# NVlabs/FoundationPose

Measured on AMD Instinct MI355X. Metric: pose-hypotheses/sec (raster+refine+score), 252 hyp x 160x160 @ 640x480 RGB-D, higher is better.
Workload: dtype f16

## Files before the change

### foundationpose_amd/_lib.py

```python
import ctypes as C
import os

import torch

_HERE = os.path.dirname(os.path.abspath(__file__))
LIB_PATH = os.environ.get("FP_AMD_LIB") or os.path.join(_HERE, "csrc", "libfp_amd.so")
ABI_VERSION = 234
_lib = None

vp, ci, cf, cd, sz = C.c_void_p, C.c_int, C.c_float, C.c_double, C.c_size_t

SIGNATURES = {
    "fp_last_error": (C.c_char_p, []),
    "fp_version": (ci, []),
    "fp_mesh_create": (ci, [vp, vp, vp, vp, vp, vp, vp, ci, ci, ci, ci, C.POINTER(vp)]),
    "fp_mesh_destroy": (None, [vp]),
    "fp_mesh_set_create": (ci, [vp, ci, C.POINTER(vp)]),
    "fp_mesh_set_destroy": (None, [vp]),
    "fp_mesh_set_workspace_bytes": (sz, [vp, ci, ci, ci]),
    "fp_depth_erode": (ci, [vp, vp, ci, ci, ci, cf, cf, cf, vp]),
    "fp_depth_bilateral": (ci, [vp, vp, ci, ci, ci, cf, cf, cf, vp]),
    "fp_depth_to_xyz": (ci, [vp, vp, cf, ci, vp, ci, ci, vp]),
    "fp_crop_windows": (ci, [vp, vp, vp, vp, ci, cd, vp, vp, ci, cd, ci, ci, ci, vp, vp, vp]),
    "fp_depth_erode_frames": (ci, [vp, vp, ci, ci, ci, ci, cf, cf, cf, vp]),
# ... 22 lines not shown
    "fp_tsdf_count_triangles": (ci, [vp, vp, ci, ci, ci, cf, vp, vp]),
    "fp_tsdf_emit_triangles": (ci, [vp, vp, vp, vp, ci, ci, ci, vp, cf, cf, vp, C.c_longlong, vp, vp, vp, vp, vp]),
    "fp_tsdf_label_components": (ci, [vp, ci, ci, ci, vp, vp, vp]),
    "fp_tsdf_raycast": (ci, [vp, vp, vp, vp, ci, ci, ci, vp, cf, cf, vp, vp, vp, vp, ci, vp, ci, ci, ci, ci, ci, cf, cf, cf, vp, vp, vp, vp, vp]),
    "fp_texture_bake": (ci, [vp, ci, vp, ci, vp, vp, vp, vp, vp, vp, ci, ci, ci, ci, ci, cf, cf, cf, vp, vp, vp]),
    "fp_workspace_bytes": (sz, [ci, ci, ci, ci, ci]),
    "fp_raster_lds_bytes": (sz, [ci]),
    "fp_render_crops": (ci, [vp, vp, vp, vp, cf, vp, vp, vp, vp, vp, ci, ci, ci, ci, ci, ci, cf, cf, cf, ci, vp, vp, vp, vp, vp, vp, vp, vp, sz, vp]),
    "fp_warp_crops": (ci, [vp, vp, vp, vp, vp, vp, vp, ci, vp, cf, vp, vp, ci, ci, ci, ci, ci, ci, ci, ci, vp, vp]),
    "fp_pose_update": (ci, [vp, vp, vp, ci, ci, vp, cf, cf, vp, vp, ci, ci, vp, vp, vp, ci, vp, vp, vp, ci, vp, cf, vp]),
    "fp_conv7x7s2_bn_relu_fwd": (ci, [vp, vp, vp, vp, vp, vp, ci, ci, ci, ci, vp]),
    "fp_igemm_f16_fwd": (ci, [vp, vp, vp, vp, vp, ci, ci, ci, ci, vp, vp]),
    "fp_pack_conv3x3_tiles_f16": (ci, [vp, vp, ci, ci, vp]),
    "fp_pack_conv3x3_tiles_direct_f16": (ci, [vp, vp, ci, ci, vp]),
    "fp_conv3x3_sw_lds_bytes": (ci, []),
    "fp_igemm_splitk_workspace_bytes": (sz, [ci, ci, ci]),
    "fp_igemm_f16_splitk_fwd": (ci, [vp, vp, vp, vp, vp, ci, ci, ci, ci, vp, ci, vp, sz, vp]),
    "fp_add_pe_f16_fwd": (ci, [vp, vp, vp, ci, ci, ci, vp]),
    "fp_replicate_rows_f16": (ci, [vp, vp, ci, ci, ci, ci, ci, C.c_longlong, vp]),
    "fp_replicate_segments_f16": (ci, [vp, vp, ci, ci, ci, ci, ci, C.c_longlong, vp]),
    "fp_layernorm_res_fwd": (ci, [vp, vp, vp, ci, vp, vp, vp, cf, vp, vp, ci, ci, vp]),
    "fp_pack_linear512_f16": (ci, [vp, vp, vp]),
    "fp_linear512_f16_fwd": (ci, [vp, vp, vp, vp, ci, ci, ci, vp]),
    "fp_linear_layernorm_fwd": (ci, [vp, vp, vp, vp, vp, vp, ci, vp, vp, cf, vp, vp, ci, ci, ci, ci, vp]),
    "fp_ffn_layernorm_mean_fwd": (ci, [vp, vp, vp, vp, vp, vp, vp, vp, cf, vp, vp, C.c_size_t, ci, ci, vp]),
    "fp_encoder_tail_workspace_bytes": (sz, [ci, ci]),
    "fp_encoder_tail_mean_fwd": (ci, [vp, ci, vp, vp, vp, vp, vp, vp, vp, vp, vp, vp, vp, vp, cf, vp, vp, sz, ci, ci, vp]),
    "fp_colmean_f16_fwd": (ci, [vp, vp, vp, vp, cf, vp, ci, ci, ci, vp]),
    "fp_rows_linear_fwd": (ci, [vp, vp, vp, vp, ci, ci, ci, ci, vp]),
    "fp_attention_f16_fwd": (ci, [vp, vp, ci, ci, ci, ci, ci, vp]),
    "fp_attention_segments_f16_fwd": (ci, [vp, vp, vp, ci, ci, ci, ci, ci, vp]),
    "fp_cluster_poses": (ci, [cf, cf, vp, ci, vp, ci, vp]),
}


class FpAmdError(RuntimeError):
    pass


def lib():
    global _lib
    if _lib is None:
        if not os.path.exists(LIB_PATH):
            raise FpAmdError(
                f"{LIB_PATH} is missing: the HIP extension is not built (run __graft_entry__.build() or "
                f"`make -C foundationpose_amd/csrc`). There is no CPU fallback.")
# ... 18 lines not shown
```

### foundationpose_amd/csrc/linear_ln.hip

```cpp
#include <hip/hip_fp16.h>
#include <stdlib.h>
#include <string.h>
#include <type_traits>
#include "igemm_common.h"
#include "rowops_ln.h"

#ifdef FP_PROFILE_BUILD
__device__ unsigned long long ll_dbg[8];
extern "C" int fp_dbg_linear_ln(unsigned long long* out, int reset) {
  if (reset) { unsigned long long z[8] = {0, 0, 0, 0, 0, 0, ~0ull, 0}; return (int)hipMemcpyToSymbol(HIP_SYMBOL(ll_dbg), z, sizeof(z)); }
  return (int)hipMemcpyFromSymbol(out, HIP_SYMBOL(ll_dbg), 8 * sizeof(unsigned long long));
}
#define LL_CLK(t) const unsigned long long t = wall_clock64()
#else
#define LL_CLK(t)
#endif

namespace {

constexpr int LL_BM = 128, LL_BN = 512, LL_K = 512, LL_NW = 8, LL_THREADS = LL_NW * 64, LL_BK = 32;
constexpr int LL_NK = LL_K / LL_BK;
constexpr int LL_KK = LL_BK / 16;
constexpr int LL_TM = LL_BM / 32;
constexpr int LL_ROWB = LL_BK * 2;
// ... 7 lines not shown

struct LinearLnParams {
  const _Float16* X;
  const _Float16* Wp;
  const float* bias;
  const float* x32;
  const _Float16* tok16;
  const float* pe;
  int S;
  const float* gamma;
  const float* beta;
  float eps;
  float* y32;
  _Float16* y16;
  int M;
  int ldx;
  float* part;
  const _Float16* W2p;
  const float* bias2;
  const _Float16* W1p;
  const float* bias1;
};

__global__ __launch_bounds__(256) void k_pack_w512(const _Float16* __restrict__ W, _Float16* __restrict__ out, int K) {
  const int o = blockIdx.x * 256 + threadIdx.x;
  const int lane = o & 63, i = (o >> 6) & 1, rest = o >> 7, nq = K / 16;
  const int q = rest % nq, w = rest / nq;
  if (w >= LL_BN / 64) return;
  const half8 v = *reinterpret_cast<const half8*>(W + (size_t)(64 * w + 32 * i + (lane & 31)) * K + 16 * q + 8 * (lane >> 5));
  *reinterpret_cast<half8*>(out + (size_t)o * 8) = v;
}

__device__ __forceinline__ int ll_swz(int row) { return (row >> 2) & 3; }

__device__ __forceinline__ void ll_dma16(const __amdgpu_buffer_rsrc_t& rs, void* lds, int voff, int soff) {
  __builtin_amdgcn_raw_ptr_buffer_load_lds(rs, (__attribute__((address_space(3))) void*)lds, 16, voff, soff, 0, 0);
}

__device__ __forceinline__ void ll_wait_vm(int n) {
  switch (n) {
    case 0: asm volatile("s_waitcnt vmcnt(0)" ::: "memory"); break;
    case 1: asm volatile("s_waitcnt vmcnt(1)" ::: "memory"); break;
    case 2: asm volatile("s_waitcnt vmcnt(2)" ::: "memory"); break;
    case 4: asm volatile("s_waitcnt vmcnt(4)" ::: "memory"); break;
    case 5: asm volatile("s_waitcnt vmcnt(5)" ::: "memory"); break;
    case 6: asm volatile("s_waitcnt vmcnt(6)" ::: "memory"); break;
    case 8: asm volatile("s_waitcnt vmcnt(8)" ::: "memory"); break;
    case 9: asm volatile("s_waitcnt vmcnt(9)" ::: "memory"); break;
    case 10: asm volatile("s_waitcnt vmcnt(10)" ::: "memory"); break;
    default: asm volatile("s_waitcnt vmcnt(0)" ::: "memory"); break;
  }
}
// ... 295 lines not shown
    const int mrow = m0 + wid * LL_ROWS_PER_WAVE;
    if (mrow < p.M) store8f(p.part + (size_t)(mrow / LL_ROWS_PER_WAVE) * 512 + lane * 8, csum);
  }
#ifdef FP_PROFILE_BUILD
  asm volatile("s_waitcnt vmcnt(0)" ::: "memory");
  LL_CLK(t_end);
  if (tid == 0) {
    atomicAdd(&ll_dbg[0], t_loop1 - t_start); atomicAdd(&ll_dbg[1], t_loop2 - t_pre); atomicAdd(&ll_dbg[2], t_park - t_loop2);
    atomicAdd(&ll_dbg[3], t_end - t_park); atomicAdd(&ll_dbg[4], 1ull); atomicMin(&ll_dbg[6], t_start); atomicMax(&ll_dbg[7], t_end);
  }
#endif
}

struct Linear512Params {
  const _Float16* X;
  const _Float16* Wp;
  const float* bias;
  _Float16* Y;
  int M, N, relu;
};
constexpr int L5_XBUF = 32 * 64;
constexpr int L5_BIAS_OFF = LL_E_BYTES + LL_NW * L5_XBUF;
constexpr int L5_MAX_N = 3072;
constexpr int l5_lds(int N) { return L5_BIAS_OFF + N * 4; }
static_assert(l5_lds(L5_MAX_N) <= 160 * 1024, "tile does not fit the 160 KiB LDS");

__global__ __launch_bounds__(LL_THREADS, 1) void k_linear512(Linear512Params p) {
  extern __shared__ __attribute__((aligned(16))) unsigned char smem[];
  const int tid = threadIdx.x, lane = tid & 63;
  const int wid = __builtin_amdgcn_readfirstlane(tid >> 6);
  float* bias_lds = reinterpret_cast<float*>(smem + L5_BIAS_OFF);
  unsigned char* xbuf = smem + LL_E_BYTES + wid * L5_XBUF;
  const int m0 = blockIdx.x * LL_BM;
  const int nblk = p.N / LL_BN;

  for (int q = wid; q < p.N / 256; q += LL_NW) {
    float* dst = bias_lds + q * 256;
    if (p.bias) {
      const __amdgpu_buffer_rsrc_t rs = __builtin_amdgcn_make_buffer_rsrc(const_cast<float*>(p.bias), 0, p.N * 4, 0x00020000);
      ll_dma16(rs, dst, lane * 16, q * 1024);
    } else {
      *reinterpret_cast<float4_*>(dst + lane * 4) = float4_{0.f, 0.f, 0.f, 0.f};
    }
  }
  unsigned aoff32;
  {
    const int row = wid * 16 + lane / 4;
    const int c = (lane % 4) ^ ll_swz(row);
    int m = m0 + row;
    m = m < p.M ? m : p.M - 1;
    aoff32 = (unsigned)(((size_t)m * LL_K + c * 8) * 2);
  }
  const __amdgpu_buffer_rsrc_t rsA = __builtin_amdgcn_make_buffer_rsrc(const_cast<_Float16*>(p.X), 0, 0x7FFFFFFF, 0x00020000);
  auto request_a = [&](int ks) { ll_dma16(rsA, smem + ks * LL_A_BLOCK + wid * 1024, (int)aoff32, ks * (LL_BK * 2)); };
  half8 wr[LL_LW + 1][LL_KK][2];
  auto request_w = [&](const _Float16* wp, int ks, int slot) {
    const _Float16* src = wp + ((size_t)wid * (LL_K / 16) + ks * LL_KK) * 1024 + lane * 8;
#pragma unroll
    for (int kk = 0; kk < LL_KK; ++kk)
#pragma unroll
      for (int i = 0; i < 2; ++i) wr[slot][kk][i] = *reinterpret_cast<const half8*>(src + (kk * 2 + i) * 512);
  };
  float16_ acc[2][LL_TM];
  const int frow = lane & 31, fhalf = lane >> 5;
  const unsigned char* a_ptr[2][LL_KK];
#pragma unroll
  for (int kk = 0; kk < LL_KK; ++kk) {
    a_ptr[0][kk] = smem + frow * LL_ROWB + (((2 * kk + fhalf) ^ ll_swz(frow)) << 4);
    a_ptr[1][kk] = a_ptr[0][kk] + 8 * LL_A_BLOCK;
  }
  half8 fa[2][LL_TM];
  auto read_a = [&](int ks, int kk, int slot) {
#pragma unroll
    for (int t = 0; t < LL_TM; ++t)
      fa[slot][t] = *reinterpret_cast<const half8*>(a_ptr[ks >> 3][kk] + (ks & 7) * LL_A_BLOCK + t * 32 * LL_ROWB);
  };
  auto mfma_group = [&](int wslot, int kk, int aslot) {
#pragma unroll
    for (int i = 0; i < 2; ++i)
#pragma unroll
      for (int j = 0; j < LL_TM; ++j)
        acc[i][j] = __builtin_amdgcn_mfma_f32_32x32x16_f16(wr[wslot][kk][i], fa[aslot][j], acc[i][j], 0, 0, 0);
  };
  auto zero_acc = [&]() {
#pragma unroll
    for (int i = 0; i < 2; ++i)
#pragma unroll
      for (int j = 0; j < LL_TM; ++j)
#pragma unroll
        for (int e = 0; e < 16; ++e) acc[i][j][e] = 0.f;
  };
  auto store_block = [&](int nb) {
    const half4 zero4 = {0, 0, 0, 0};
#pragma unroll
    for (int i = 0; i < 2; ++i) {
      const int nl = nb * LL_BN + wid * 64 + i * 32;
#pragma unroll
      for (int j = 0; j < LL_TM; ++j) {
#pragma unroll
        for (int g = 0; g < 4; ++g) {
          const float4_ bv = *reinterpret_cast<const float4_*>(bias_lds + nl + 8 * g + 4 * fhalf);
          half4 v;
#pragma unroll
          for (int e = 0; e < 4; ++e) v[e] = (_Float16)(acc[i][j][g * 4 + e] + bv[e]);
          if (p.relu) v = __builtin_elementwise_max(v, zero4);
          *reinterpret_cast<half4*>(xbuf + frow * 64 + ((g ^ ll_swz(frow)) << 4) + 8 * fhalf) = v;
        }
        __builtin_amdgcn_s_waitcnt(0xc07f);
        __builtin_amdgcn_wave_barrier();
#pragma unroll
        for (int h = 0; h < 2; ++h) {
          const int r = h * 16 + (lane >> 2), c = lane & 3;
          const half8 o = *reinterpret_cast<const half8*>(xbuf + r * 64 + ((c ^ ll_swz(r)) << 4));
          const int m = m0 + j * 32 + r;
          if (m < p.M) *reinterpret_cast<half8*>(p.Y + (size_t)m * p.N + nl + c * 8) = o;
        }
        __builtin_amdgcn_s_waitcnt(0xc07f);
        __builtin_amdgcn_wave_barrier();
      }
    }
  };

  zero_acc();
#pragma unroll
  for (int j = 0; j < LL_LA - LL_LW; ++j) request_a(j);
#pragma unroll
  for (int j = 0; j < LL_LW; ++j) { request_a(j + LL_LA - LL_LW); request_w(p.Wp, j, j); }
  ll_wait_vm(ll_after_w(0));
  __builtin_amdgcn_s_barrier();
  read_a(0, 0, 0);
#pragma unroll
  for (int ks = 0; ks < LL_NK; ++ks) {
    if (ks + LL_LA < LL_NK) request_a(ks + LL_LA);
    if (ks + LL_LW < LL_NK) request_w(p.Wp, ks + LL_LW, (ks + LL_LW) % (LL_LW + 1));
    read_a(ks, 1, 1);
    __builtin_amdgcn_sched_barrier(0);
    mfma_group(ks % (LL_LW + 1), 0, 0);
    __builtin_amdgcn_sched_barrier(0);
    if (ks + 1 < LL_NK) {
      ll_wait_vm(ll_after_w(ks + 1));
      __builtin_amdgcn_s_barrier();
      read_a(ks + 1, 0, 0);
    }
// ... 9 lines not shown
#pragma unroll 1
  for (int nb = 1; nb < nblk; ++nb) {
    const _Float16* wp = p.Wp + (size_t)nb * LL_BN * LL_K;
    zero_acc();
    read_a(0, 0, 0);
#pragma unroll
    for (int ks = 0; ks < LL_NK; ++ks) {
      if (ks + LL_LW < LL_NK) request_w(wp, ks + LL_LW, (ks + LL_LW) % (LL_LW + 1));
      read_a(ks, 1, 1);
      __builtin_amdgcn_sched_barrier(0);
      mfma_group(ks % (LL_LW + 1), 0, 0);
      __builtin_amdgcn_sched_barrier(0);
      if (ks + 1 < LL_NK) read_a(ks + 1, 0, 0);
      __builtin_amdgcn_sched_barrier(0);
      mfma_group(ks % (LL_LW + 1), 1, 1);
      __builtin_amdgcn_sched_barrier(0);
    }
    if (nb + 1 < nblk) {
#pragma unroll
      for (int j = 0; j < LL_LW; ++j) request_w(wp + (size_t)LL_BN * LL_K, j, j);
    }
    store_block(nb);
  }
}

__global__ __launch_bounds__(512) void k_ln_mean_finish(const float* __restrict__ part, const float* __restrict__ gamma,
                                                       const float* __restrict__ beta, float* __restrict__ out, int S) {
  const int g = blockIdx.x, c = threadIdx.x;
  const int nch = S / 16;
  const float* src = part + (size_t)g * nch * 512 + c;
  float a = 0.f;
  for (int k = 0; k < nch; ++k) a += src[(size_t)k * 512];
  a *= 1.0f / (float)S;
  out[(size_t)g * 512 + c] = fmaf(a, gamma[c], beta[c]);
}

}

extern "C" int fp_pack_linear512_f16(const void* w16, void* packed, void* stream) {
  FP_REQUIRE(w16 && packed, "fp_pack_linear512_f16: NULL tensor");
  FP_REQUIRE(w16 != packed, "fp_pack_linear512_f16: cannot pack in place");
  FP_REQUIRE((((size_t)w16 | (size_t)packed) & 15) == 0, "fp_pack_linear512_f16: tensors must be 16-byte aligned");
  hipLaunchKernelGGL(k_pack_w512, dim3(LL_BN * LL_K / 8 / 256), dim3(256), 0, (hipStream_t)stream, (const _Float16*)w16, (_Float16*)packed,
                     LL_K);
  FP_CHECK_LAUNCH("fp_pack_linear512_f16");
  return FP_OK;
}

extern "C" int fp_linear512_f16_fwd(const void* x16, const void* w_packed, const float* bias, void* y16, int M, int N, int relu,
                                    void* stream) {
  FP_REQUIRE(M >= 0, "fp_linear512_f16_fwd: M < 0");
  if (M == 0) return FP_OK;
  FP_REQUIRE(x16 && w_packed && y16, "fp_linear512_f16_fwd: NULL tensor");
  FP_REQUIRE(N >= LL_BN && N % LL_BN == 0 && N <= L5_MAX_N, "fp_linear512_f16_fwd: N=%d must be a multiple of 512, at most %d", N, L5_MAX_N);
  FP_REQUIRE((long long)M * N < (1ll << 31), "fp_linear512_f16_fwd: output exceeds 2^31 elements");
  FP_REQUIRE((((size_t)x16 | (size_t)w_packed | (size_t)bias | (size_t)y16) & 15) == 0, "fp_linear512_f16_fwd: tensors must be 16-byte aligned");
  Linear512Params p;
  p.X = (const _Float16*)x16; p.Wp = (const _Float16*)w_packed; p.bias = bias; p.Y = (_Float16*)y16; p.M = M; p.N = N; p.relu = relu ? 1 : 0;
  const int lds = l5_lds(N);
  FP_SET_MAX_LDS(k_linear512, l5_lds(L5_MAX_N));
  hipLaunchKernelGGL(k_linear512, dim3(fp_cdiv(M, LL_BM)), dim3(LL_THREADS), lds, (hipStream_t)stream, p);
  FP_CHECK_LAUNCH("fp_linear512_f16_fwd");
  return FP_OK;
}

extern "C" int fp_ffn_layernorm_mean_fwd(const void* y16, const void* w1_packed, const float* b1, const void* w2_packed, const float* b2,
                                         const float* x32, const float* gamma, const float* beta, float eps, float* out,
                                         float* workspace, size_t workspace_bytes, int groups, int rows_per_group, void* stream) {
  FP_REQUIRE(groups >= 0, "fp_ffn_layernorm_mean_fwd: groups < 0");
  if (groups == 0) return FP_OK;
  FP_REQUIRE(y16 && w1_packed && w2_packed && x32 && gamma && beta && out && workspace, "fp_ffn_layernorm_mean_fwd: NULL tensor");
  FP_REQUIRE(rows_per_group >= 16 && rows_per_group % 16 == 0,
             "fp_ffn_layernorm_mean_fwd: rows_per_group=%d must be a multiple of 16 (a wave sums 16 consecutive rows, which have to belong to one group)", rows_per_group);
  const long long M = (long long)groups * rows_per_group;
  FP_REQUIRE(M * 512 < (1ll << 30), "fp_ffn_layernorm_mean_fwd: operands exceed 2 GiB");
  FP_REQUIRE((((size_t)y16 | (size_t)w1_packed | (size_t)w2_packed | (size_t)b1 | (size_t)b2 | (size_t)x32 | (size_t)gamma | (size_t)beta) & 15) == 0,
             "fp_ffn_layernorm_mean_fwd: tensors must be 16-byte aligned");
  const int tiles = fp_cdiv((int)M, LL_BM);
  FP_REQUIRE(workspace_bytes >= (size_t)(M / 16) * 512 * sizeof(float), "fp_ffn_layernorm_mean_fwd: workspace too small");
  LinearLnParams p;
  p.X = (const _Float16*)y16; p.Wp = (const _Float16*)w1_packed; p.bias = b1; p.x32 = x32; p.tok16 = nullptr; p.pe = nullptr;
  p.S = rows_per_group; p.gamma = gamma; p.beta = beta; p.eps = eps; p.y32 = nullptr; p.y16 = nullptr; p.M = (int)M; p.ldx = LL_K;
  p.part = workspace; p.W2p = (const _Float16*)w2_packed; p.bias2 = b2; p.W1p = nullptr; p.bias1 = nullptr;
  FP_SET_MAX_LDS((k_rows512<true, true>), LL_LDS);
  hipLaunchKernelGGL((k_rows512<true, true>), dim3(tiles), dim3(LL_THREADS), LL_LDS, (hipStream_t)stream, p);
  hipLaunchKernelGGL(k_ln_mean_finish, dim3(groups), dim3(512), 0, (hipStream_t)stream, (const float*)workspace, gamma, beta, out,
// ... 69 lines not shown
```

### foundationpose_amd/engine.py

```python
import contextlib

import torch
import torch.nn.functional as F

from . import ops

USE_MIOPEN = False


FUSED_OUT_PROJ_LN = True


FUSED_FFN = True


ROWS_QKV = True
ROWS_QKV_MIN_ROWS = 4096
PACKED_CONV_TILES = True
MERGED_HEAD_QKV = True
FUSED_TAIL = True
CONV_MFMA_16X16X32 = True
SPECIALIZED_EPILOGUE = True
CONV_DIRECT_STORE = True


def _conv_backend():
    if USE_MIOPEN or not torch.backends.cudnn.is_available():
        return contextlib.nullcontext()
    return torch.backends.cudnn.flags(enabled=False)


def _bn_affine(sd, bn_p):
    if bn_p is None or (bn_p + ".weight") not in sd:
        return None, None
    scale = sd[bn_p + ".weight"].float() / torch.sqrt(sd[bn_p + ".running_var"].float() + 1e-5)
    shift = sd[bn_p + ".bias"].float() - sd[bn_p + ".running_mean"].float() * scale
    return scale.contiguous(), shift.contiguous()


def _r16(t):
    return t.to(torch.float16).to(torch.float32).contiguous()


class _Conv:

    def __init__(self, sd, conv_p, bn_p, stride, dtype, channels_last):
# ... 76 lines not shown

    def __call__(self, x):
        x = F.layer_norm(x + self.att(x), (x.shape[-1],), self.n1[0], self.n1[1], 1e-5)
        ff = F.linear(F.relu(F.linear(x, *self.l1)), *self.l2)
        return F.layer_norm(x + ff, (x.shape[-1],), self.n2[0], self.n2[1], 1e-5)


def _conv_params(sd, conv_p, bn_p, second_output=False):
    w = sd[conv_p + ".weight"].float()
    b = sd.get(conv_p + ".bias")
    scale, shift = _bn_affine(sd, bn_p)
    wk = w.permute(0, 2, 3, 1).reshape(w.shape[0], -1).to(torch.float16).contiguous()
    tiles, direct = None, bool(CONV_DIRECT_STORE and CONV_MFMA_16X16X32 and SPECIALIZED_EPILOGUE and b is not None and not second_output)
    if wk.is_cuda and w.shape[2] == 3 and w.shape[3] == 3 and w.shape[0] % 128 == 0 and w.shape[1] % 32 == 0 and PACKED_CONV_TILES:
        tiles = (ops.pack_conv3x3_tiles_direct if direct else ops.pack_conv3x3_tiles)(wk, w.shape[0], w.shape[1])
    return dict(w=wk, w_tiles=tiles, tiles_direct=direct and tiles is not None, bias=None if b is None else _r16(b.float()), scale=scale, shift=shift)


SPLITK_MAX_HYPS = 12
HEADS_TWO_STREAMS_MAX_HYPS = 12
SPLITK_TARGET_WGS = 384
SMALL_CALL_CEILING = 31

_SWITCHES = ("FUSED_OUT_PROJ_LN", "FUSED_FFN", "ROWS_QKV", "PACKED_CONV_TILES", "MERGED_HEAD_QKV", "FUSED_TAIL", "CONV_MFMA_16X16X32", "SPECIALIZED_EPILOGUE", "CONV_DIRECT_STORE", "SPLITK_MAX_HYPS", "HEADS_TWO_STREAMS_MAX_HYPS")


@contextlib.contextmanager
def overrides(**kw):
    g = globals()
    for k, v in kw.items():
        if k not in _SWITCHES:
            raise KeyError(f"engine.overrides: unknown switch {k!r} (known: {', '.join(_SWITCHES)})")
        if k.endswith("_MAX_HYPS") and not (0 <= int(v) <= SMALL_CALL_CEILING):
            raise ValueError(f"engine.overrides: {k} = {v} is outside 0..{SMALL_CALL_CEILING}")
    saved = {k: g[k] for k in kw}
    g.update(kw)
    try:
        yield
    finally:
        g.update(saved)


def small_call(n, limit):
    return n <= min(int(limit), SMALL_CALL_CEILING)


def splitk_pieces(rows, cout, cin):
# ... 108 lines not shown
        No = self.w.shape[0]
        y = torch.empty((M, No), dtype=torch.float16, device=x.device)
        Gm = ops.IgemmGeom.matrix
        ops.igemm_f16(x2, Gm(K), self.w, self.b, y, Gm(No), M, No, K, 1, relu=relu)
        return y.reshape(*x.shape[:-1], No)


class _HipRowsLinear:

    def __init__(self, w, b):
        self.w = w.to(torch.float16).contiguous()
        self.b = _r16(b.float())

    def __call__(self, x, round_f16=True, out_f16=False, out=None):
        return ops.rows_linear(x, self.w, self.b, round_f16=round_f16, out_f16=out_f16, out=out)


class _HipMHA:
    def __init__(self, sd, p, fp16_scores, nhead=4, small_calls=True):
        self.qkv = _HipLinear(sd[p + ".in_proj_weight"], sd[p + ".in_proj_bias"])
        self.out = _HipLinear(sd[p + ".out_proj.weight"], sd[p + ".out_proj.bias"])
        self.out_rows = _HipRowsLinear(sd[p + ".out_proj.weight"], sd[p + ".out_proj.bias"])
        self.nhead, self.fp16_scores = nhead, fp16_scores
        self.qkv_p = ops.PackedLinear512(self.qkv.w) if tuple(self.qkv.w.shape) == (1536, 512) else None
        self.small_calls = small_calls
        self._sk = {}

    def context(self, x16, slot=0, small_calls=True):
        Bn, L, D = x16.shape
        qkv = self.in_proj(x16, slot, small_calls)
        return ops.attention_f16(qkv.reshape(Bn, L, 3 * D), self.nhead, fp16_scores=self.fp16_scores)

    def in_proj(self, x16, slot=0, small_calls=True):
        Bn, L, D = x16.shape
        if ROWS_QKV and self.qkv_p is not None and Bn * L >= ROWS_QKV_MIN_ROWS:
            qkv = ops.linear512(x16, self.qkv_p, self.qkv.b)
        elif self.small_calls and small_calls and small_call(Bn, SPLITK_MAX_HYPS) and D % 64 == 0 and D // 64 >= 4:
            M, No = Bn * L, self.qkv.w.shape[0]
            pieces = max(1, min(D // 64 // 2, round(SPLITK_TARGET_WGS / (-(-M // 128) * (No // 128)))))
            key = (M, No, pieces, x16.device, slot)
            ws = self._sk.get(key)
            if ws is None:
                ws = self._sk[key] = torch.empty(ops.igemm_splitk_workspace_bytes(M, No, pieces), dtype=torch.uint8, device=x16.device)
            qkv = torch.empty((M, No), dtype=torch.float16, device=x16.device)
            Gm = ops.IgemmGeom.matrix
            ops.igemm_f16_splitk(x16.reshape(M, D), Gm(D), self.qkv.w, self.qkv.b, qkv, Gm(No), M, No, D, 1, pieces, ws)
        else:
# ... 42 lines not shown
    return {k: v.detach().to(device) for k, v in sd.items()}


class RefinePlan:
    small_calls = True

    def __init__(self, model, device, precision="fp16", channels_last=True):
        _check_precision(precision)
        self.dtype = torch.float16 if precision == "fp16" else torch.float32
        self.hip = self.dtype == torch.float16
        self.module = model if precision == "torch_amp" else None
        if self.module is not None:
            return
        sd = _dev_sd(model, device)
        self.heads = {}
        if self.hip:
            self.enc = _HipEncoder(sd, "encodeA", "encodeAB", device)
            for name in ("trans", "rot"):
                self.heads[name] = (_HipEncoderLayer(sd, f"{name}_head.0"),
                                    _HipRowsLinear(sd[f"{name}_head.1.weight"], sd[f"{name}_head.1.bias"]))
            wt, wr = (self.heads[n][0].att.qkv for n in ("trans", "rot"))
            if tuple(wt.w.shape) == (1536, 512) and tuple(wr.w.shape) == (1536, 512):
                cut = lambda t: (t[0:512], t[512:1024], t[1024:1536])
                self.qkv2_p = ops.PackedLinear512(torch.cat([p for pair in zip(cut(wt.w), cut(wr.w)) for p in pair], 0).contiguous())
                self.qkv2_b = torch.cat([p for pair in zip(cut(wt.b), cut(wr.b)) for p in pair], 0).contiguous()
            else:
                self.qkv2_p = None
        else:
            self.enc = _Encoder(sd, "encodeA", "encodeAB", self.dtype, channels_last)
            for name in ("trans", "rot"):
                self.heads[name] = (_TorchEncoderLayer(sd, f"{name}_head.0", self.dtype),
                                    sd[f"{name}_head.1.weight"].to(self.dtype), sd[f"{name}_head.1.bias"].to(self.dtype))

    def _head_side_stream(self, tok16):
        if not getattr(self, "two_stream_heads", True) or not self.small_calls or not small_call(tok16.shape[0], HEADS_TWO_STREAMS_MAX_HYPS) \
                or tok16.device.type != "cuda" or ops.KernelTimers.active is not None:
            return None
        from . import overlap
        if torch.cuda.is_current_stream_capturing() and not overlap.reserved(tok16.device, 1):
            return None
        if not overlap.side_streams_overlap(tok16.device, 1):
            return None
        return overlap.reserve_streams(tok16.device, 1)[0]

    @torch.inference_mode()
    def __call__(self, AB, slot=0, shared_b=False):
        out = {}
# ... 123 lines not shown
```

### foundationpose_amd/ops.py

```python
import ctypes as C
from typing import NamedTuple, Optional

import numpy as np
import torch

from . import _lib

FLAG_NORMALIZE_XYZ = 1
FLAG_OUT_F16 = 2
MODE_REFINE = 0
MODE_SCORE = 1
ROT_AXIS_ANGLE = 0
ROT_6D = 1
TRANS_TRACKNET, TRANS_DEEPIM, TRANS_RAW = 0, 1, 2


def _stream(t=None):
    if t is None:
        return C.c_void_p(torch.cuda.current_stream().cuda_stream)
    dev = t.device
    if dev.index is not None and dev.index != torch.cuda.current_device():
        raise _lib.FpAmdError(f"tensor on {dev} but the current device is cuda:{torch.cuda.current_device()}: wrap the call in "
                              f"`with torch.cuda.device({dev.index}):` (kernels launch on the current device)")
    return C.c_void_p(torch.cuda.current_stream(dev).cuda_stream)
# ... 1778 lines not shown
    _, Hp, Wp, Ct = (int(v) for v in buf.shape)
    st = _lib.lib().fp_replicate_segments_f16(C.c_void_p(buf.data_ptr() + 2 * int(c0)), _ptr(segments.dev), len(segments), n, Hp * Wp,
                                              int(c1) - int(c0), Ct, Hp * Wp * Ct, _stream(buf))
    _lib.check(st, "fp_replicate_segments_f16")
    return buf


def layernorm_res(branch16, gamma, beta, eps=1e-5, x32=None, tok16=None, pe=None, want32=True, want16=True):
    br = _dev(branch16, torch.float16, "branch16")
    D = int(br.shape[-1])
    M = br.numel() // D
    x32 = _dev(x32, torch.float32, "x32"); tok16 = _dev(tok16, torch.float16, "tok16"); pe = _dev(pe, torch.float32, "pe")
    S = int(pe.shape[-2]) if pe is not None else 0
    y32 = torch.empty(br.shape, dtype=torch.float32, device=br.device) if want32 else None
    y16 = torch.empty_like(br) if want16 else None
    st = _lib.lib().fp_layernorm_res_fwd(_ptr(x32), _ptr(tok16), _ptr(pe), S, _ptr(br), _ptr(_dev(gamma, torch.float32, "gamma")),
                                         _ptr(_dev(beta, torch.float32, "beta")), float(eps), _ptr(y32), _ptr(y16), M, D, _stream(br))
    _lib.check(st, "fp_layernorm_res_fwd")
    return y32, y16


class PackedLinear512:

    def __init__(self, w16):
        w = _dev(w16, torch.float16, "w16")
        if w.dim() != 2 or int(w.shape[1]) != 512 or int(w.shape[0]) % 512 or int(w.shape[0]) == 0:
            raise _lib.FpAmdError(f"PackedLinear512: weight {tuple(w.shape)}, must be (512 n, 512)")
        self.out_features = int(w.shape[0])
        self.data = torch.empty_like(w)
        for blk in range(self.out_features // 512):
            _lib.check(_lib.lib().fp_pack_linear512_f16(_ptr(w[blk * 512:]), _ptr(self.data[blk * 512:]), _stream(w)), "fp_pack_linear512_f16")


def _packed(w, name, out_features=512):
    if not isinstance(w, PackedLinear512):
        raise _lib.FpAmdError(f"{name}: the weight must be a PackedLinear512 (ops.PackedLinear512(w16))")
    if out_features is not None and w.out_features != out_features:
        raise _lib.FpAmdError(f"{name}: packed weight has {w.out_features} output features, expected {out_features}")
    return w.data


def linear512(x16, w_packed, bias, relu=False, out=None):
    x = _dev(x16, torch.float16, "x16")
    w = _packed(w_packed, "linear512", None)
    if int(x.shape[-1]) != 512:
        raise _lib.FpAmdError(f"linear512: x16 (..., {int(x.shape[-1])}), must be (..., 512)")
    N = w_packed.out_features
    M = x.numel() // 512
    y = out if out is not None else torch.empty(tuple(x.shape[:-1]) + (N,), dtype=torch.float16, device=x.device)
    if y.dtype != torch.float16 or y.numel() != M * N or not y.is_contiguous():
        raise _lib.FpAmdError("linear512: out must be a contiguous fp16 tensor of M x N elements")
    _lib.check(_lib.lib().fp_linear512_f16_fwd(_ptr(x), _ptr(w), _ptr(_dev(bias, torch.float32, "bias")), _ptr(y), M, N, 1 if relu else 0,
                                               _stream(x)), "fp_linear512_f16_fwd")
    return y


def linear_layernorm_res(x16, w_packed, bias, gamma, beta, eps=1e-5, x32=None, tok16=None, pe=None, want32=True, want16=True):
    w = _packed(w_packed, "linear_layernorm_res")
    if not (torch.is_tensor(x16) and x16.is_cuda and x16.dtype == torch.float16):
        raise _lib.FpAmdError("linear_layernorm_res: x16 must be a CUDA float16 tensor")
    K = int(x16.shape[-1])
    D = 512
    if K != 512:
        raise _lib.FpAmdError(f"linear_layernorm_res: x16 (..., {K}), must be (..., 512)")
    M = x16.numel() // K
    x, ldx = x16, _column_block(x16, "linear_layernorm_res: x16", sep="")
    x32 = _dev(x32, torch.float32, "x32"); tok16 = _dev(tok16, torch.float16, "tok16"); pe = _dev(pe, torch.float32, "pe")
    S = int(pe.shape[-2]) if pe is not None else 0
    shape = tuple(x.shape[:-1]) + (D,)
    y32 = torch.empty(shape, dtype=torch.float32, device=x.device) if want32 else None
    y16 = torch.empty(shape, dtype=torch.float16, device=x.device) if want16 else None
    st = _lib.lib().fp_linear_layernorm_fwd(_ptr(x), _ptr(w), _ptr(_dev(bias, torch.float32, "bias")), _ptr(x32), _ptr(tok16), _ptr(pe), S,
                                            _ptr(_dev(gamma, torch.float32, "gamma")), _ptr(_dev(beta, torch.float32, "beta")), float(eps),
                                            _ptr(y32), _ptr(y16), M, K, D, ldx, _stream(x))
    _lib.check(st, "fp_linear_layernorm_fwd")
    return y32, y16
# ... 301 lines not shown
```

### include/fp_amd.h

```cpp
#ifndef FP_AMD_H
#define FP_AMD_H

#include <stddef.h>
#include <stdint.h>

#ifdef __cplusplus
extern "C" {
#endif

typedef enum {
  FP_OK = 0,
  FP_ERR_INVALID_ARG = -1,
  FP_ERR_WORKSPACE = -2,
  FP_ERR_LAUNCH = -3,
  FP_ERR_UNSUPPORTED = -4
} fp_status;

#define FP_FLAG_NORMALIZE_XYZ 1
#define FP_FLAG_OUT_F16 2

#define FP_MODE_REFINE 0
#define FP_MODE_SCORE 1

#define FP_ROT_AXIS_ANGLE 0
// ... 209 lines not shown
size_t fp_igemm_splitk_workspace_bytes(int M, int N, int splits);
int fp_igemm_f16_splitk_fwd(const void* x , const fp_igemm_geom* x_geom , const void* w , void* y ,
                            const fp_igemm_geom* y_geom , int M, int N, int Cin, int taps,
                            const fp_igemm_epilogue* epilogue , int splits, void* workspace ,
                            size_t workspace_bytes, void* stream);

int fp_add_pe_f16_fwd(const void* tok , const float* pe , void* out , int M, int S, int D, void* stream);

int fp_replicate_rows_f16(const void* src , void* dst , int copies, int rows, int channels, int src_row_stride,
                          int dst_row_stride, long long dst_copy_stride, void* stream);

int fp_replicate_segments_f16(void* buf , const int32_t* seg_offsets , int segments, int images, int pixels,
                              int channels, int pixel_stride, long long image_stride, void* stream);

int fp_layernorm_res_fwd(const float* x32 , const void* tok16 , const float* pe , int S,
                         const void* branch16 , const float* gamma , const float* beta , float eps,
                         float* y32 , void* y16 , int M, int D, void* stream);

int fp_pack_linear512_f16(const void* w16 , void* packed , void* stream);

int fp_linear512_f16_fwd(const void* x16 , const void* w_packed , const float* bias , void* y16 ,
                         int M, int N, int relu, void* stream);

int fp_linear_layernorm_fwd(const void* x16 , const void* w16_packed , const float* bias ,
                            const float* x32 , const void* tok16 , const float* pe , int S,
                            const float* gamma , const float* beta , float eps, float* y32 ,
                            void* y16 , int M, int K, int D, int ldx ,
                            void* stream);

size_t fp_encoder_tail_workspace_bytes(int groups, int rows_per_group);
int fp_encoder_tail_mean_fwd(const void* ctx16 , int ldx, const void* wo_packed , const float* bo ,
                             const void* tok16 , const float* pe , const float* gamma1 , const float* beta1 ,
                             const void* w1_packed , const float* b1 , const void* w2_packed ,
                             const float* b2 , const float* gamma2 , const float* beta2 , float eps,
                             float* out , void* workspace , size_t workspace_bytes, int groups, int rows_per_group,
                             void* stream);

int fp_ffn_layernorm_mean_fwd(const void* y16 , const void* w1_packed , const float* b1 ,
                              const void* w2_packed , const float* b2 , const float* x32 ,
                              const float* gamma , const float* beta , float eps, float* out ,
                              float* workspace , size_t workspace_bytes, int groups, int rows_per_group, void* stream);

int fp_colmean_f16_fwd(const void* x , const float* resid32 , const float* gamma ,
                       const float* beta , float eps, float* out , int groups, int rows_per_group,
                       int D, void* stream);

// ... 24 lines not shown
```

Measured before the change: 7996.

## Add direct-store variant of linear512 with swapped MFMA operands and packed weight order

Measured after the change: 8077 (median of 6 runs). 1.01x the previous value.

```diff
diff --git a/foundationpose_amd/_lib.py b/foundationpose_amd/_lib.py
--- a/foundationpose_amd/_lib.py
+++ b/foundationpose_amd/_lib.py
@@ -68,6 +68,8 @@
     "fp_layernorm_res_fwd": (ci, [vp, vp, vp, ci, vp, vp, vp, cf, vp, vp, ci, ci, vp]),
     "fp_pack_linear512_f16": (ci, [vp, vp, vp]),
     "fp_linear512_f16_fwd": (ci, [vp, vp, vp, vp, ci, ci, ci, vp]),
+    "fp_pack_linear512_direct_f16": (ci, [vp, vp, vp]),
+    "fp_linear512_flags_f16_fwd": (ci, [vp, vp, vp, vp, ci, ci, ci, vp]),
     "fp_linear_layernorm_fwd": (ci, [vp, vp, vp, vp, vp, vp, ci, vp, vp, cf, vp, vp, ci, ci, ci, ci, vp]),
     "fp_ffn_layernorm_mean_fwd": (ci, [vp, vp, vp, vp, vp, vp, vp, vp, cf, vp, vp, C.c_size_t, ci, ci, vp]),
     "fp_encoder_tail_workspace_bytes": (sz, [ci, ci]),
diff --git a/foundationpose_amd/csrc/linear_ln.hip b/foundationpose_amd/csrc/linear_ln.hip
--- a/foundationpose_amd/csrc/linear_ln.hip
+++ b/foundationpose_amd/csrc/linear_ln.hip
@@ -53,12 +53,13 @@
   const float* bias1;
 };
 
-__global__ __launch_bounds__(256) void k_pack_w512(const _Float16* __restrict__ W, _Float16* __restrict__ out, int K) {
+__global__ __launch_bounds__(256) void k_pack_w512(const _Float16* __restrict__ W, _Float16* __restrict__ out, int K, int direct) {
   const int o = blockIdx.x * 256 + threadIdx.x;
   const int lane = o & 63, i = (o >> 6) & 1, rest = o >> 7, nq = K / 16;
   const int q = rest % nq, w = rest / nq;
   if (w >= LL_BN / 64) return;
-  const half8 v = *reinterpret_cast<const half8*>(W + (size_t)(64 * w + 32 * i + (lane & 31)) * K + 16 * q + 8 * (lane >> 5));
+  const int row = direct ? 2 * (lane & 31) + i : 32 * i + (lane & 31);
+  const half8 v = *reinterpret_cast<const half8*>(W + (size_t)(64 * w + row) * K + 16 * q + 8 * (lane >> 5));
   *reinterpret_cast<half8*>(out + (size_t)o * 8) = v;
 }
 
@@ -400,17 +401,30 @@
 constexpr int L5_XBUF = 32 * 64;
 constexpr int L5_BIAS_OFF = LL_E_BYTES + LL_NW * L5_XBUF;
 constexpr int L5_MAX_N = 3072;
-constexpr int l5_lds(int N) { return L5_BIAS_OFF + N * 4; }
+constexpr int l5_lds(int N, bool direct = false) { return (direct ? LL_E_BYTES : L5_BIAS_OFF) + N * 4; }
 static_assert(l5_lds(L5_MAX_N) <= 160 * 1024, "tile does not fit the 160 KiB LDS");
 
-__global__ __launch_bounds__(LL_THREADS, 1) void k_linear512(Linear512Params p) {
+#ifdef FP_PROFILE_BUILD
+__device__ unsigned long long l5_dbg[4];
+extern "C" int fp_dbg_linear512(unsigned long long* out, int reset) {
+  if (reset) { unsigned long long z[4] = {0, 0, 0, 0}; return (int)hipMemcpyToSymbol(HIP_SYMBOL(l5_dbg), z, sizeof(z)); }
+  return (int)hipMemcpyFromSymbol(out, HIP_SYMBOL(l5_dbg), 4 * sizeof(unsigned long long));
+}
+#endif
+
+template <bool DIRECT, bool FULL>
+__device__ __forceinline__ void l5_body(const Linear512Params& p) {
   extern __shared__ __attribute__((aligned(16))) unsigned char smem[];
   const int tid = threadIdx.x, lane = tid & 63;
   const int wid = __builtin_amdgcn_readfirstlane(tid >> 6);
-  float* bias_lds = reinterpret_cast<float*>(smem + L5_BIAS_OFF);
+  float* bias_lds = reinterpret_cast<float*>(smem + (DIRECT ? LL_E_BYTES : L5_BIAS_OFF));
   unsigned char* xbuf = smem + LL_E_BYTES + wid * L5_XBUF;
   const int m0 = blockIdx.x * LL_BM;
   const int nblk = p.N / LL_BN;
+#ifdef FP_PROFILE_BUILD
+  const unsigned long long l5_t0 = wall_clock64();
+  unsigned long long l5_ts = 0;
+#endif
 
   for (int q = wid; q < p.N / 256; q += LL_NW) {
     float* dst = bias_lds + q * 256;
@@ -457,18 +471,51 @@
 #pragma unroll
     for (int i = 0; i < 2; ++i)
 #pragma unroll
+      for (int j = 0; j < LL_TM; ++j) {
+        if constexpr (DIRECT) acc[i][j] = __builtin_amdgcn_mfma_f32_32x32x16_f16(fa[aslot][j], wr[wslot][kk][i], acc[i][j], 0, 0, 0);
+        else acc[i][j] = __builtin_amdgcn_mfma_f32_32x32x16_f16(wr[wslot][kk][i], fa[aslot][j], acc[i][j], 0, 0, 0);
+      }
+  };
+  auto zero_acc = [&]() {
+#pragma unroll
+    for (int i = 0; i < 2; ++i)
+#pragma unroll
       for (int j = 0; j < LL_TM; ++j)
-        acc[i][j] = __builtin_amdgcn_mfma_f32_32x32x16_f16(wr[wslot][kk][i], fa[aslot][j], acc[i][j], 0, 0, 0);
-  };
-  auto zero_acc = [&]() {
-#pragma unroll
-    for (int i = 0; i < 2; ++i)
-#pragma unroll
-      for (int j = 0; j < LL_TM; ++j)
 #pragma unroll
         for (int e = 0; e < 16; ++e) acc[i][j][e] = 0.f;
   };
-  auto store_block = [&](int nb) {
+  typedef _Float16 half2_ __attribute__((ext_vector_type(2)));
+  const __amdgpu_buffer_rsrc_t rsY = __builtin_amdgcn_make_buffer_rsrc(p.Y, 0, DIRECT ? p.M * p.N * 2 : 0, 0x00020000);
+  const int row_bytes = p.N * 2;
+  const int yoff = (4 * fhalf) * row_bytes + (64 * wid + 2 * frow) * 2;
+  const int rows_left = p.M - m0 - 4 * fhalf;
+  auto store_block_direct = [&](int nb) {
+    typedef float float2_ __attribute__((ext_vector_type(2)));
+    const float2_ bv = *reinterpret_cast<const float2_*>(bias_lds + nb * LL_BN + 64 * wid + 2 * frow);
+    const int voff = yoff + nb * (LL_BN * 2);
+    const half2_ zero2 = {0, 0};
+    unsigned soff = (unsigned)m0 * (unsigned)row_bytes;
+    asm volatile("" : "+s"(soff));
+    int left = rows_left;
+#pragma unroll
+    for (int j = 0; j < LL_TM; ++j) {
+#pragma unroll
+      for (int r = 0; r < 16; ++r) {
+        const int row = 32 * j + (r & 3) + 8 * (r >> 2);
+        half2_ v = {(_Float16)(acc[0][j][r] + bv[0]), (_Float16)(acc[1][j][r] + bv[1])};
+        if (p.relu) v = __builtin_elementwise_max(v, zero2);
+        const unsigned vu = __builtin_bit_cast(unsigned, v);
+        if constexpr (FULL) {
+          __builtin_amdgcn_raw_buffer_store_b32(vu, rsY, voff, (int)soff, 0);
+        } else {
+          asm volatile("" : "+v"(left));
+          if (row < left) __builtin_amdgcn_raw_buffer_store_b32(vu, rsY, voff, (int)soff, 0);
+        }
+        soff += (r & 3) == 3 ? 5u * (unsigned)row_bytes : (unsigned)row_bytes;
+      }
+    }
+  };
+  auto store_block_lds = [&](int nb) {
     const half4 zero4 = {0, 0, 0, 0};
 #pragma unroll
     for (int i = 0; i < 2; ++i) {
@@ -497,6 +544,16 @@
         __builtin_amdgcn_wave_barrier();
       }
     }
+  };
+  auto store_block = [&](int nb) {
+#ifdef FP_PROFILE_BUILD
+    const unsigned long long ts0 = wall_clock64();
+#endif
+    if constexpr (DIRECT) store_block_direct(nb);
+    else store_block_lds(nb);
+#ifdef FP_PROFILE_BUILD
+    l5_ts += wall_clock64() - ts0;
+#endif
   };
 
   zero_acc();
@@ -552,6 +609,18 @@
     }
     store_block(nb);
   }
+#ifdef FP_PROFILE_BUILD
+  if (tid == 0) {
+    atomicAdd(&l5_dbg[0], l5_ts); atomicAdd(&l5_dbg[1], wall_clock64() - l5_t0); atomicAdd(&l5_dbg[2], 1ull);
+    atomicAdd(&l5_dbg[3], (unsigned long long)nblk);
+  }
+#endif
+}
+
+__global__ __launch_bounds__(LL_THREADS, 1) void k_linear512(Linear512Params p) { l5_body<false, false>(p); }
+__global__ __launch_bounds__(LL_THREADS, 1) void k_linear512_direct(Linear512Params p) {
+  if ((int)(blockIdx.x + 1) * LL_BM <= p.M) l5_body<true, true>(p);
+  else l5_body<true, false>(p);
 }
 
 __global__ __launch_bounds__(512) void k_ln_mean_finish(const float* __restrict__ part, const float* __restrict__ gamma,
@@ -572,26 +641,56 @@
   FP_REQUIRE(w16 != packed, "fp_pack_linear512_f16: cannot pack in place");
   FP_REQUIRE((((size_t)w16 | (size_t)packed) & 15) == 0, "fp_pack_linear512_f16: tensors must be 16-byte aligned");
   hipLaunchKernelGGL(k_pack_w512, dim3(LL_BN * LL_K / 8 / 256), dim3(256), 0, (hipStream_t)stream, (const _Float16*)w16, (_Float16*)packed,
-                     LL_K);
+                     LL_K, 0);
   FP_CHECK_LAUNCH("fp_pack_linear512_f16");
   return FP_OK;
 }
 
+extern "C" int fp_pack_linear512_direct_f16(const void* w16, void* packed, void* stream) {
+  FP_REQUIRE(w16 && packed, "fp_pack_linear512_direct_f16: NULL tensor");
+  FP_REQUIRE(w16 != packed, "fp_pack_linear512_direct_f16: cannot pack in place");
+  FP_REQUIRE((((size_t)w16 | (size_t)packed) & 15) == 0, "fp_pack_linear512_direct_f16: tensors must be 16-byte aligned");
+  hipLaunchKernelGGL(k_pack_w512, dim3(LL_BN * LL_K / 8 / 256), dim3(256), 0, (hipStream_t)stream, (const _Float16*)w16, (_Float16*)packed,
+                     LL_K, 1);
+  FP_CHECK_LAUNCH("fp_pack_linear512_direct_f16");
+  return FP_OK;
+}
+
+static int l5_launch(const char* who, const void* x16, const void* w_packed, const float* bias, void* y16, int M, int N, int flags,
+                     void* stream) {
+  FP_REQUIRE(M >= 0, "%s: M < 0", who);
+  FP_REQUIRE((flags & ~(FP_LINEAR512_RELU | FP_LINEAR512_DIRECT_STORE | FP_LINEAR512_W_DIRECT)) == 0, "%s: unknown flags 0x%x", who, flags);
+  const bool direct = (flags & FP_LINEAR512_DIRECT_STORE) != 0, w_direct = (flags & FP_LINEAR512_W_DIRECT) != 0;
+  FP_REQUIRE(w_direct == direct, "%s: w_packed is in the row order of %s but this launch runs %s (FP_LINEAR512_W_DIRECT, FP_LINEAR512_DIRECT_STORE)",
+             who, w_direct ? "fp_pack_linear512_direct_f16" : "fp_pack_linear512_f16", direct ? "k_linear512_direct" : "k_linear512");
+  if (M == 0) return FP_OK;
+  FP_REQUIRE(x16 && w_packed && y16, "%s: NULL tensor", who);
+  FP_REQUIRE(N >= LL_BN && N % LL_BN == 0 && N <= L5_MAX_N, "%s: N=%d must be a multiple of 512, at most %d", who, N, L5_MAX_N);
+  FP_REQUIRE((long long)M * N < (1ll << 31), "%s: output exceeds 2^31 elements", who);
+  FP_REQUIRE(!direct || (long long)M * N * 2 < (1ll << 31), "%s: FP_LINEAR512_DIRECT_STORE needs an output below 2 GiB (M=%d N=%d)", who, M, N);
+  FP_REQUIRE((((size_t)x16 | (size_t)w_packed | (size_t)bias | (size_t)y16) & 15) == 0, "%s: tensors must be 16-byte aligned", who);
+  Linear512Params p;
+  p.X = (const _Float16*)x16; p.Wp = (const _Float16*)w_packed; p.bias = bias; p.Y = (_Float16*)y16; p.M = M; p.N = N;
+  p.relu = (flags & FP_LINEAR512_RELU) ? 1 : 0;
+  if (direct) {
+    FP_SET_MAX_LDS(k_linear512_direct, l5_lds(L5_MAX_N, true));
+    hipLaunchKernelGGL(k_linear512_direct, dim3(fp_cdiv(M, LL_BM)), dim3(LL_THREADS), l5_lds(N, true), (hipStream_t)stream, p);
+  } else {
+    FP_SET_MAX_LDS(k_linear512, l5_lds(L5_MAX_N));
+    hipLaunchKernelGGL(k_linear512, dim3(fp_cdiv(M, LL_BM)), dim3(LL_THREADS), l5_lds(N), (hipStream_t)stream, p);
+  }
+  FP_CHECK_LAUNCH(who);
+  return FP_OK;
+}
+
 extern "C" int fp_linear512_f16_fwd(const void* x16, const void* w_packed, const float* bias, void* y16, int M, int N, int relu,
                                     void* stream) {
-  FP_REQUIRE(M >= 0, "fp_linear512_f16_fwd: M < 0");
-  if (M == 0) return FP_OK;
-  FP_REQUIRE(x16 && w_packed && y16, "fp_linear512_f16_fwd: NULL tensor");
-  FP_REQUIRE(N >= LL_BN && N % LL_BN == 0 && N <= L5_MAX_N, "fp_linear512_f16_fwd: N=%d must be a multiple of 512, at most %d", N, L5_MAX_N);
-  FP_REQUIRE((long long)M * N < (1ll << 31), "fp_linear512_f16_fwd: output exceeds 2^31 elements");
-  FP_REQUIRE((((size_t)x16 | (size_t)w_packed | (size_t)bias | (size_t)y16) & 15) == 0, "fp_linear512_f16_fwd: tensors must be 16-byte aligned");
-  Linear512Params p;
-  p.X = (const _Float16*)x16; p.Wp = (const _Float16*)w_packed; p.bias = bias; p.Y = (_Float16*)y16; p.M = M; p.N = N; p.relu = relu ? 1 : 0;
-  const int lds = l5_lds(N);
-  FP_SET_MAX_LDS(k_linear512, l5_lds(L5_MAX_N));
-  hipLaunchKernelGGL(k_linear512, dim3(fp_cdiv(M, LL_BM)), dim3(LL_THREADS), lds, (hipStream_t)stream, p);
-  FP_CHECK_LAUNCH("fp_linear512_f16_fwd");
-  return FP_OK;
+  return l5_launch("fp_linear512_f16_fwd", x16, w_packed, bias, y16, M, N, relu ? FP_LINEAR512_RELU : 0, stream);
+}
+
+extern "C" int fp_linear512_flags_f16_fwd(const void* x16, const void* w_packed, const float* bias, void* y16, int M, int N, int flags,
+                                          void* stream) {
+  return l5_launch("fp_linear512_flags_f16_fwd", x16, w_packed, bias, y16, M, N, flags, stream);
 }
 
 extern "C" int fp_ffn_layernorm_mean_fwd(const void* y16, const void* w1_packed, const float* b1, const void* w2_packed, const float* b2,
diff --git a/foundationpose_amd/engine.py b/foundationpose_amd/engine.py
--- a/foundationpose_amd/engine.py
+++ b/foundationpose_amd/engine.py
@@ -22,6 +22,7 @@
 CONV_MFMA_16X16X32 = True
 SPECIALIZED_EPILOGUE = True
 CONV_DIRECT_STORE = True
+LINEAR512_DIRECT_STORE = True
 
 
 def _conv_backend():
@@ -144,7 +145,7 @@
 SPLITK_TARGET_WGS = 384
 SMALL_CALL_CEILING = 31
 
-_SWITCHES = ("FUSED_OUT_PROJ_LN", "FUSED_FFN", "ROWS_QKV", "PACKED_CONV_TILES", "MERGED_HEAD_QKV", "FUSED_TAIL", "CONV_MFMA_16X16X32", "SPECIALIZED_EPILOGUE", "CONV_DIRECT_STORE", "SPLITK_MAX_HYPS", "HEADS_TWO_STREAMS_MAX_HYPS")
+_SWITCHES = ("FUSED_OUT_PROJ_LN", "FUSED_FFN", "ROWS_QKV", "PACKED_CONV_TILES", "MERGED_HEAD_QKV", "FUSED_TAIL", "CONV_MFMA_16X16X32", "SPECIALIZED_EPILOGUE", "CONV_DIRECT_STORE", "LINEAR512_DIRECT_STORE","SPLITK_MAX_HYPS", "HEADS_TWO_STREAMS_MAX_HYPS")
 
 
 @contextlib.contextmanager
@@ -299,7 +300,7 @@
         self.out = _HipLinear(sd[p + ".out_proj.weight"], sd[p + ".out_proj.bias"])
         self.out_rows = _HipRowsLinear(sd[p + ".out_proj.weight"], sd[p + ".out_proj.bias"])
         self.nhead, self.fp16_scores = nhead, fp16_scores
-        self.qkv_p = ops.PackedLinear512(self.qkv.w) if tuple(self.qkv.w.shape) == (1536, 512) else None
+        self.qkv_p = ops.PackedLinear512(self.qkv.w, direct=LINEAR512_DIRECT_STORE) if tuple(self.qkv.w.shape) == (1536, 512) else None
         self.small_calls = small_calls
         self._sk = {}
 
@@ -388,7 +389,8 @@
             wt, wr = (self.heads[n][0].att.qkv for n in ("trans", "rot"))
             if tuple(wt.w.shape) == (1536, 512) and tuple(wr.w.shape) == (1536, 512):
                 cut = lambda t: (t[0:512], t[512:1024], t[1024:1536])
-                self.qkv2_p = ops.PackedLinear512(torch.cat([p for pair in zip(cut(wt.w), cut(wr.w)) for p in pair], 0).contiguous())
+                self.qkv2_p = ops.PackedLinear512(torch.cat([p for pair in zip(cut(wt.w), cut(wr.w)) for p in pair], 0).contiguous(),
+                                                     direct=LINEAR512_DIRECT_STORE)
                 self.qkv2_b = torch.cat([p for pair in zip(cut(wt.b), cut(wr.b)) for p in pair], 0).contiguous()
             else:
                 self.qkv2_p = None
diff --git a/foundationpose_amd/ops.py b/foundationpose_amd/ops.py
--- a/foundationpose_amd/ops.py
+++ b/foundationpose_amd/ops.py
@@ -1824,14 +1824,25 @@
 
 class PackedLinear512:
 
-    def __init__(self, w16):
+    def __init__(self, w16, direct=False):
         w = _dev(w16, torch.float16, "w16")
         if w.dim() != 2 or int(w.shape[1]) != 512 or int(w.shape[0]) % 512 or int(w.shape[0]) == 0:
             raise _lib.FpAmdError(f"PackedLinear512: weight {tuple(w.shape)}, must be (512 n, 512)")
         self.out_features = int(w.shape[0])
+        self.direct = bool(direct)
+        self.w16, self._other = w, None
         self.data = torch.empty_like(w)
+        fn, name = (_lib.lib().fp_pack_linear512_direct_f16, "fp_pack_linear512_direct_f16") if self.direct else \
+                   (_lib.lib().fp_pack_linear512_f16, "fp_pack_linear512_f16")
         for blk in range(self.out_features // 512):
-            _lib.check(_lib.lib().fp_pack_linear512_f16(_ptr(w[blk * 512:]), _ptr(self.data[blk * 512:]), _stream(w)), "fp_pack_linear512_f16")
+            _lib.check(fn(_ptr(w[blk * 512:]), _ptr(self.data[blk * 512:]), _stream(w)), name)
+
+    def in_order(self, direct):
+        if bool(direct) == self.direct:
+            return self
+        if self._other is None:
+            self._other = PackedLinear512(self.w16, direct=direct)
+        return self._other
 
 
 def _packed(w, name, out_features=512):
@@ -1839,21 +1850,34 @@
         raise _lib.FpAmdError(f"{name}: the weight must be a PackedLinear512 (ops.PackedLinear512(w16))")
     if out_features is not None and w.out_features != out_features:
         raise _lib.FpAmdError(f"{name}: packed weight has {w.out_features} output features, expected {out_features}")
+    if w.direct and name != "linear512":
+        raise _lib.FpAmdError(f"{name}: the weight is packed in the row order of linear512's direct-store kernel (PackedLinear512(w16, direct=True)); "
+                              "the row-owning fused kernels read the plain order")
     return w.data
 
 
-def linear512(x16, w_packed, bias, relu=False, out=None):
+LINEAR512_RELU = 1
+LINEAR512_DIRECT_STORE = 2
+LINEAR512_W_DIRECT = 4
+
+
+def linear512(x16, w_packed, bias, relu=False, out=None, direct_store=None):
     x = _dev(x16, torch.float16, "x16")
-    w = _packed(w_packed, "linear512", None)
     if int(x.shape[-1]) != 512:
         raise _lib.FpAmdError(f"linear512: x16 (..., {int(x.shape[-1])}), must be (..., 512)")
+    _packed(w_packed, "linear512", None)
     N = w_packed.out_features
     M = x.numel() // 512
+    if direct_store is None:
+        from . import engine
+        direct_store = bool(engine.LINEAR512_DIRECT_STORE) and M * N * 2 < 2 ** 31
+        w_packed = w_packed.in_order(direct_store)
     y = out if out is not None else torch.empty(tuple(x.shape[:-1]) + (N,), dtype=torch.float16, device=x.device)
     if y.dtype != torch.float16 or y.numel() != M * N or not y.is_contiguous():
         raise _lib.FpAmdError("linear512: out must be a contiguous fp16 tensor of M x N elements")
-    _lib.check(_lib.lib().fp_linear512_f16_fwd(_ptr(x), _ptr(w), _ptr(_dev(bias, torch.float32, "bias")), _ptr(y), M, N, 1 if relu else 0,
-                                               _stream(x)), "fp_linear512_f16_fwd")
+    flags = (LINEAR512_RELU if relu else 0) | (LINEAR512_DIRECT_STORE if direct_store else 0) | (LINEAR512_W_DIRECT if w_packed.direct else 0)
+    _lib.check(_lib.lib().fp_linear512_flags_f16_fwd(_ptr(x), _ptr(w_packed.data), _ptr(_dev(bias, torch.float32, "bias")), _ptr(y), M, N, flags,
+                                                     _stream(x)), "fp_linear512_flags_f16_fwd")
     return y
 
 
diff --git a/include/fp_amd.h b/include/fp_amd.h
--- a/include/fp_amd.h
+++ b/include/fp_amd.h
@@ -255,6 +255,14 @@
 int fp_linear512_f16_fwd(const void* x16 , const void* w_packed , const float* bias , void* y16 ,
                          int M, int N, int relu, void* stream);
 
+int fp_pack_linear512_direct_f16(const void* w16 , void* packed , void* stream);
+
+#define FP_LINEAR512_RELU 1
+#define FP_LINEAR512_DIRECT_STORE 2
+#define FP_LINEAR512_W_DIRECT 4
+int fp_linear512_flags_f16_fwd(const void* x16 , const void* w_packed , const float* bias , void* y16 ,
+                               int M, int N, int flags, void* stream);
+
 int fp_linear_layernorm_fwd(const void* x16 , const void* w16_packed , const float* bias ,
                             const float* x32 , const void* tok16 , const float* pe , int S,
                             const float* gamma , const float* beta , float eps, float* y32 ,
```
